# zwyang6/ExCEL

Hardware: AMD Instinct MI355X
Metric: images/sec (CAM+PAR refine, 448x448) (higher is better)
Workload: dtype bf16x3 (fp32 as bf16 hi+lo, fp32 accumulate)

## Files before the change

excel_amd/csrc/attn.hip:

```cpp
#include <stdlib.h>
#include "common.h"
#include "excel_internal.h"

namespace EXCEL_SPLIT_NS {

#define HD 64

struct RowpassArgs {
    float* out;
    float2* stats;
    int B, H, N;
    float scale;
    const unsigned short* qkvs;
    int flash_nq;
    int xcd_local;
    int tail_grp;
};

typedef unsigned short u16;

template <bool FLASH>
__device__ __forceinline__ void rowpass_body_bf(const RowpassArgs& p, float* smem, int b, int h, int type, int qblk) {
    constexpr int KT_EL = 32 * 128;
    constexpr int VSUB = 1152;
    constexpr int VT_EL = 8 * VSUB / 2;
    constexpr int STAGE_EL = KT_EL + (FLASH ? VT_EL : 0);
    constexpr int PER_WAVE = FLASH ? 4 : 2;
    const int tid = threadIdx.x, lane = tid & 63;
    const int wave = __builtin_amdgcn_readfirstlane(tid >> 6);
    const int r = lane & 31, kh = lane >> 5;
    const int N = p.N;
    const int tx = (type == 0 || type == 1) ? 0 : (type == 2 ? 1 : 2);
    const int ty = (type == 0) ? 1 : tx;
    const u16* Xsp = p.qkvs + (((long long)b * 3 + tx) * p.H + h) * (long long)N * 128;
    const u16* Ysp = p.qkvs + (((long long)b * 3 + ty) * p.H + h) * (long long)N * 128;
    const u16* Vsp = p.qkvs + (((long long)b * 3 + 2) * p.H + h) * (long long)N * 128;
    u16* ring = reinterpret_cast<u16*>(smem);
    const unsigned ring_b = __builtin_amdgcn_readfirstlane(lds_addr(ring));

    const int q0 = qblk * 128 + wave * 32;
    const int qrow = min(q0 + r, N - 1);
    splitx8 xh[4], xl[4];
#pragma unroll
    for (int s4 = 0; s4 < 4; ++s4) {
        xh[s4] = *reinterpret_cast<const splitx8*>(Xsp + (long long)qrow * 128 + s4 * 16 + kh * 8);
        xl[s4] = *reinterpret_cast<const splitx8*>(Xsp + (long long)qrow * 128 + 64 + s4 * 16 + kh * 8);
    }

    asm volatile("" : "+v"(xh[0]), "+v"(xh[1]), "+v"(xh[2]), "+v"(xh[3]), "+v"(xl[0]), "+v"(xl[1]), "+v"(xl[2]), "+v"(xl[3]));
    typedef __attribute__((address_space(3))) unsigned char* lds_bptr;
    const long long kplane_bytes = (long long)N * 256;
    const long long kavail = ((((long long)p.B * 3 - ((long long)b * 3 + ty)) * p.H - h) * kplane_bytes);
    const __amdgpu_buffer_rsrc_t rs_k = __builtin_amdgcn_make_buffer_rsrc((void*)Ysp, 0, (int)(kavail < (1LL << 31) - 1 ? kavail : (1LL << 31) - 1), 0x00020000);
    const long long vavail = ((((long long)p.B * 3 - ((long long)b * 3 + 2)) * p.H - h) * kplane_bytes);
    const __amdgpu_buffer_rsrc_t rs_v = __builtin_amdgcn_make_buffer_rsrc((void*)Vsp, 0, FLASH ? (int)(vavail < (1LL << 31) - 1 ? vavail : (1LL << 31) - 1) : 0, 0x00020000);
    int koffb[2], voffb[2];
#pragma unroll
    for (int j = 0; j < 2; ++j) {
        const int krow = wave * 8 + j * 4 + (lane >> 4);
        koffb[j] = krow * 256 + (((lane & 15) ^ (krow & 15)) * 16);
        const int sub = wave * 2 + j;
        voffb[j] = (lane >> 1) * 256 + (sub >> 2) * 128 + (((sub & 3) * 16 + (lane & 1) * 8) * 2);
    }
    auto issue_piece = [&](int kt, int stage, int idx) {
        unsigned dstk = __builtin_amdgcn_readfirstlane(ring_b + stage * (STAGE_EL * 2));
        asm volatile("" : "+s"(dstk));
        if (idx < 2) {
            __builtin_amdgcn_raw_ptr_buffer_load_lds(rs_k, (lds_bptr)(unsigned long long)(dstk + (wave * 8 + idx * 4) * 256), 16, koffb[idx], kt * (32 * 256), 0, 0);
        } else if (FLASH) {
            const int j = idx - 2;
            __builtin_amdgcn_raw_ptr_buffer_load_lds(rs_v, (lds_bptr)(unsigned long long)(dstk + KT_EL * 2 + (wave * 2 + j) * VSUB), 16, voffb[j], kt * (32 * 256), 0, 0);
        }
    };
    auto issue = [&](int kt, int stage) {
#pragma unroll
        for (int idx = 0; idx < PER_WAVE; ++idx) issue_piece(kt, stage, idx);
    };

    const float c2 = p.scale * 1.4426950408889634f;
    float m = -INFINITY, l = 0.f;
    f32x16 oT[2];
#pragma unroll
    for (int e = 0; e < 16; ++e) { oT[0][e] = 0.f; oT[1][e] = 0.f; }

    const int nkt = (N + 31) / 32;
    issue(0, 0);
    if (nkt > 1) issue(1, 1);
    int stage = 0;
    for (int kt = 0; kt < nkt; ++kt) {
        if (kt + 1 < nkt) {
            if (PER_WAVE == 4) asm volatile("s_waitcnt vmcnt(4)" ::: "memory");
            else asm volatile("s_waitcnt vmcnt(2)" ::: "memory");
        } else {
            asm volatile("s_waitcnt vmcnt(0)" ::: "memory");
        }
        __builtin_amdgcn_s_barrier();
        const int rstage = stage == 0 ? 2 : stage - 1;
        const bool refill = kt + 2 < nkt;
        if (q0 >= N) {
            if (refill) issue(kt + 2, rstage);
            stage = (stage == 2) ? 0 : stage + 1;
            continue;
        }
        const unsigned kr = ring_b + (stage * STAGE_EL + r * 128) * 2;
        f32x16 s;
#pragma unroll
        for (int e = 0; e < 16; ++e) s[e] = 0.f;
        {
            splitx8 yh[4], yl[4];
#pragma unroll
            for (int s4 = 0; s4 < 4; ++s4) {
                yh[s4] = lds_read16(kr + (((s4 * 2 + kh) ^ (r & 15)) * 16));
                yl[s4] = lds_read16(kr + (((8 + s4 * 2 + kh) ^ (r & 15)) * 16));
            }
            lds_wait8(yh, yl);
#pragma unroll
            for (int s4 = 0; s4 < 4; ++s4) {
                if (refill && s4 < PER_WAVE) issue_piece(kt + 2, rstage, s4);
                s = EXCEL_MFMA16(yl[s4], xh[s4], s, 0, 0, 0);
                s = EXCEL_MFMA16(yh[s4], xl[s4], s, 0, 0, 0);
                s = EXCEL_MFMA16(yh[s4], xh[s4], s, 0, 0, 0);
                __builtin_amdgcn_sched_barrier(0);
            }
        }
        if (kt == nkt - 1) {
#pragma unroll
            for (int e = 0; e < 16; ++e)
                if (kt * 32 + c32_row(e, lane) >= N) s[e] = -INFINITY;
        }
        float mx = s[0];
#pragma unroll
        for (int e = 1; e < 16; ++e) mx = fmaxf(mx, s[e]);
        {
            float mlo, mhi;
            wave_halves(mx, mlo, mhi);
            mx = fmaxf(mlo, mhi) * c2;
        }
        const float m_new = fmaxf(m, mx);
        const bool grew = m_new > m;
        const float alpha = __builtin_amdgcn_exp2f(m - m_new);
        float ps = 0.f;
#pragma unroll
        for (int e = 0; e < 16; ++e) {
            s[e] = __builtin_amdgcn_exp2f(fmaf(s[e], c2, -m_new));
            ps += s[e];
        }
        {
            float plo, phi;
            wave_halves(ps, plo, phi);
            ps = plo + phi;
        }
        l = l * alpha + ps;
        m = m_new;
        if (FLASH) {
            if (__any(grew)) {
#pragma unroll
                for (int e = 0; e < 16; ++e) { oT[0][e] *= alpha; oT[1][e] *= alpha; }
            }
            splitx8 ph[2], pl[2];
#ifdef EXCEL_SPLIT_F16
            {
                unsigned phu[2][4], plu[2][4];
#pragma unroll
                for (int e = 0; e < 16; e += 2) split_pair_bounded(s[e], s[e + 1], phu[e >> 3][(e & 7) >> 1], plu[e >> 3][(e & 7) >> 1]);
#pragma unroll
                for (int q = 0; q < 2; ++q) {
                    ph[q] = __builtin_bit_cast(splitx8, uint4{phu[q][0], phu[q][1], phu[q][2], phu[q][3]});
                    pl[q] = __builtin_bit_cast(splitx8, uint4{plu[q][0], plu[q][1], plu[q][2], plu[q][3]});
                }
            }
#else
#pragma unroll
            for (int e = 0; e < 16; ++e) {
                const float hf = __uint_as_float(__float_as_uint(s[e]) & 0xFFFF0000u);
                ph[e >> 3][e & 7] = split_hi(hf);
                pl[e >> 3][e & 7] = split_hi(s[e] - hf);
            }
#endif
            const unsigned vb = ring_b + (stage * STAGE_EL + KT_EL) * 2 + ((lane >> 4) & 1) * VSUB + (4 * kh + ((lane & 15) >> 2)) * 32 + (lane & 3) * 8;
#pragma unroll
            for (int dt = 0; dt < 2; ++dt) {
                splitx4 vq[8];
                const unsigned vbd = vb + dt * 2 * VSUB;
                vq[0] = lds_read8h_tr<0>(vbd);
                vq[1] = lds_read8h_tr<256>(vbd);
                vq[2] = lds_read8h_tr<4 * VSUB>(vbd);
                vq[3] = lds_read8h_tr<4 * VSUB + 256>(vbd);
                vq[4] = lds_read8h_tr<512>(vbd);
                vq[5] = lds_read8h_tr<512 + 256>(vbd);
                vq[6] = lds_read8h_tr<4 * VSUB + 512>(vbd);
                vq[7] = lds_read8h_tr<4 * VSUB + 512 + 256>(vbd);
                asm volatile("s_waitcnt lgkmcnt(0)" : "+v"(vq[0]), "+v"(vq[1]), "+v"(vq[2]), "+v"(vq[3]), "+v"(vq[4]), "+v"(vq[5]), "+v"(vq[6]), "+v"(vq[7])::"memory");
#pragma unroll
                for (int ks = 0; ks < 2; ++ks) {
                    const splitx4 h0 = vq[ks * 4], h1 = vq[ks * 4 + 1], l0 = vq[ks * 4 + 2], l1 = vq[ks * 4 + 3];
                    const splitx8 vh = {h0[0], h0[1], h0[2], h0[3], h1[0], h1[1], h1[2], h1[3]};
                    const splitx8 vl = {l0[0], l0[1], l0[2], l0[3], l1[0], l1[1], l1[2], l1[3]};
                    oT[dt] = EXCEL_MFMA16(vl, ph[ks], oT[dt], 0, 0, 0);
                    oT[dt] = EXCEL_MFMA16(vh, pl[ks], oT[dt], 0, 0, 0);
                    oT[dt] = EXCEL_MFMA16(vh, ph[ks], oT[dt], 0, 0, 0);
                }
            }
        }
        stage = (stage == 2) ? 0 : stage + 1;
    }

    const float linv = 1.f / l;
    if (kh == 0 && q0 + r < N)
        p.stats[(((long long)b * p.H + h) * 4 + type) * N + q0 + r] = make_float2(m, linv);

    if (FLASH) {
        __syncthreads();
        float* ob = smem + wave * (32 * 65);
#pragma unroll
        for (int dt = 0; dt < 2; ++dt)
#pragma unroll
            for (int e = 0; e < 16; ++e) ob[r * 65 + dt * 32 + c32_row(e, lane)] = oT[dt][e] * linv;
        __builtin_amdgcn_s_waitcnt(0xc07f);
        for (int qq = 0; qq < 32; ++qq) {
            const int q = q0 + qq;
            if (q >= N) break;
            const float v = ob[qq * 65 + lane];
            const split_t hi = split_hi(v);
            split_t* o = reinterpret_cast<split_t*>(p.out) + ((long long)b * N + q) * 2 * (p.H * HD) + split_off(h * HD + lane, 0);
            o[0] = hi;
            o[32] = split_hi(v - (float)hi);
        }
    }
}

__global__ __launch_bounds__(256, 2) void attn_rowpass_kernel(RowpassArgs p) {
    __shared__ __attribute__((aligned(1024))) float smem[3 * (2048 + 2304)];
    int bh, qb;
    rowpass_block_map(p.N, p.xcd_local, p.tail_grp, bh, qb);
    const int b = bh / p.H, h = bh % p.H;
    const int type = blockIdx.z;
    if (type == 0 && qb < p.flash_nq) rowpass_body_bf<true>(p, smem, b, h, 0, qb);
    else rowpass_body_bf<false>(p, smem, b, h, type, qb);
}

struct AccumArgs {
    const float2* stats;
    float* a_sum;
    float* w_aff;
    float* attn_out;
    int B, H, N, NP;
    float scale;
    float w_scale;
    float aff_scale;
    int aff_init;
    const unsigned short* qkvs;
    int dbg;
    const float* ex_attn;
    float ex_scale;
};

template <bool SURGERY>
__global__ __launch_bounds__(512, 2) void attn_accum_bf_kernel(AccumArgs p) {
    constexpr int XT = 128 * 128, YT = 64 * 128;
    constexpr int NTYPE = SURGERY ? 4 : 1;
    constexpr int TILES_EL = SURGERY ? 3 * XT + 3 * YT : 2 * (XT + YT);
    __shared__ __attribute__((aligned(1024))) u16 tiles[TILES_EL];
    __shared__ __attribute__((aligned(1024))) float2 lstats[2 * NTYPE * 128 + 32];
    const int tid = threadIdx.x, lane = tid & 63;
    const int wave = __builtin_amdgcn_readfirstlane(tid >> 6);
    const int r = lane & 31, kh = lane >> 5;
    const int wq = wave >> 1, wk = wave & 1;
    int kt = blockIdx.x, qt = blockIdx.y, b = blockIdx.z;
    if (EXCEL_DBG(p.dbg) & 8) {
        const int lin = blockIdx.x + gridDim.x * (blockIdx.y + gridDim.y * blockIdx.z);
        const int id = xcd_remap(lin, gridDim.x * gridDim.y * gridDim.z);
        kt = id % gridDim.x; qt = (id / gridDim.x) % gridDim.y; b = id / (gridDim.x * gridDim.y);
    }
    const int N = p.N;

    int rowx[4], coffx[4], rowy[2], coffy[2];
#pragma unroll
    for (int j = 0; j < 4; ++j) {
        const int row_l = wave * 16 + j * 4 + (lane >> 4);
        coffx[j] = ((lane & 15) ^ (row_l & 15)) * 8;
        rowx[j] = min(qt * 128 + row_l, N - 1);
    }
#pragma unroll
    for (int j = 0; j < 2; ++j) {
        const int row_l = wave * 8 + j * 4 + (lane >> 4);
        coffy[j] = ((lane & 15) ^ (row_l & 15)) * 8;
        rowy[j] = min(kt * 64 + row_l, N - 1);
    }
    auto issue_x = [&](int off, int typ, int h) {
        const u16* src = p.qkvs + (((long long)b * 3 + typ) * p.H + h) * (long long)N * 128;
#pragma unroll
        for (int j = 0; j < 4; ++j)
            __builtin_amdgcn_global_load_lds((const __attribute__((address_space(1))) void*)(src + (long long)rowx[j] * 128 + coffx[j]),
                                             (__attribute__((address_space(3))) void*)(tiles + off + (wave * 16 + j * 4) * 128), 16, 0, 0);
    };
    auto issue_y = [&](int off, int typ, int h) {
        const u16* src = p.qkvs + (((long long)b * 3 + typ) * p.H + h) * (long long)N * 128;
#pragma unroll
        for (int j = 0; j < 2; ++j)
            __builtin_amdgcn_global_load_lds((const __attribute__((address_space(1))) void*)(src + (long long)rowy[j] * 128 + coffy[j]),
                                             (__attribute__((address_space(3))) void*)(tiles + off + (wave * 8 + j * 4) * 128), 16, 0, 0);
    };
    auto issue_stats = [&](int h) {
        float* dst = reinterpret_cast<float*>(lstats + (h & 1) * NTYPE * 128);
#pragma unroll
        for (int j = 0; j < 2; ++j) {
            const int piece = wave * 2 + j;
            if (SURGERY || piece < 4) {
                const int ty = piece >> 2, q32 = (piece & 3) * 32 + (lane >> 1);
                const float* src = reinterpret_cast<const float*>(p.stats + (((long long)b * p.H + h) * 4 + ty) * N + min(qt * 128 + q32, N - 1)) + (lane & 1);
                __builtin_amdgcn_global_load_lds((const __attribute__((address_space(1))) void*)src,
                                                 (__attribute__((address_space(3))) void*)(dst + piece * 64), 4, 0, 0);
            } else {
                const float* src = reinterpret_cast<const float*>(p.stats + (((long long)b * p.H + h) * 4) * N + min(qt * 128 + (lane >> 1), N - 1)) + (lane & 1);
                __builtin_amdgcn_global_load_lds((const __attribute__((address_space(1))) void*)src,
                                                 (__attribute__((address_space(3))) void*)(reinterpret_cast<float*>(lstats) + 2 * NTYPE * 256), 4, 0, 0);
            }
        }
    };

    f32x16 accW, accA;
#pragma unroll
    for (int e = 0; e < 16; ++e) { accW[e] = 0.f; accA[e] = 0.f; }
    const float c2 = p.scale * 1.4426950408889634f;
    const bool last_kt = kt * 64 + wk * 32 + 32 > N;

    const bool tile_oob = (qt * 128 + wq * 32 >= N) || (kt * 64 + wk * 32 >= N);
    auto score = [&](int offY, int offX, int type, int h, f32x16& acc) {
        if ((EXCEL_DBG(p.dbg) & 1) || tile_oob) return;
        const float2 ml = lstats[((h & 1) * NTYPE + type) * 128 + wq * 32 + r];
        const u16* y16 = tiles + offY + (wk * 32 + r) * 128;
        const u16* x16 = tiles + offX + (wq * 32 + r) * 128;
        f32x16 s;
#pragma unroll
        for (int e = 0; e < 16; ++e) s[e] = 0.f;
#pragma unroll
        for (int s4 = 0; s4 < 4; ++s4) {
            const int ch = ((s4 * 2 + kh) ^ (r & 15)) * 8, cl = ((8 + s4 * 2 + kh) ^ (r & 15)) * 8;
            const splitx8 yh = *reinterpret_cast<const splitx8*>(y16 + ch), yl = *reinterpret_cast<const splitx8*>(y16 + cl);
            const splitx8 xh = *reinterpret_cast<const splitx8*>(x16 + ch), xl = *reinterpret_cast<const splitx8*>(x16 + cl);
            s = EXCEL_MFMA16(yl, xh, s, 0, 0, 0);
            s = EXCEL_MFMA16(yh, xl, s, 0, 0, 0);
            s = EXCEL_MFMA16(yh, xh, s, 0, 0, 0);
        }
        if (last_kt) {
#pragma unroll
            for (int e = 0; e < 16; ++e) {
                const int key = kt * 64 + wk * 32 + c32_row(e, lane);
                const float pr = __builtin_amdgcn_exp2f(fmaf(s[e], c2, -ml.x));
                acc[e] += (key < N) ? pr * ml.y : 0.f;
            }
        } else {
#pragma unroll
            for (int e = 0; e < 16; ++e) acc[e] = fmaf(__builtin_amdgcn_exp2f(fmaf(s[e], c2, -ml.x)), ml.y, acc[e]);
        }
    };

    if (SURGERY) {
        constexpr int XQ = 0, XK = XT, XV = 2 * XT, YQ = 3 * XT, YK = 3 * XT + YT, YV = 3 * XT + 2 * YT;
        issue_y(YQ, 0, 0);
        issue_stats(0);
        issue_x(XQ, 0, 0);
        issue_x(XK, 1, 0);
        issue_y(YK, 1, 0);
        for (int h = 0; h < p.H; ++h) {
            const bool more = h + 1 < p.H && !(EXCEL_DBG(p.dbg) & 2);
            asm volatile("s_waitcnt vmcnt(6)" ::: "memory");
            __builtin_amdgcn_s_barrier();
            if (!(EXCEL_DBG(p.dbg) & 2) || h == 0) { issue_x(XV, 2, h); issue_y(YV, 2, h); }
            score(YQ, XQ, 1, h, accA);
            if (!(EXCEL_DBG(p.dbg) & 2) || h == 0) asm volatile("s_waitcnt vmcnt(6)" ::: "memory");
            __builtin_amdgcn_s_barrier();
            if (more) { issue_y(YQ, 0, h + 1); issue_stats(h + 1); }
            score(YK, XQ, 0, h, accW);
            __builtin_amdgcn_s_barrier();
            if (more) issue_x(XQ, 0, h + 1);
            score(YK, XK, 2, h, accA);
            if (more) asm volatile("s_waitcnt vmcnt(8)" ::: "memory");
            else asm volatile("s_waitcnt vmcnt(0)" ::: "memory");
            __builtin_amdgcn_s_barrier();
            if (more) { issue_x(XK, 1, h + 1); issue_y(YK, 1, h + 1); }
            score(YV, XV, 3, h, accA);
        }
    } else {
        issue_x(0, 0, 0);
        issue_y(XT, 1, 0);
        issue_stats(0);
        for (int h = 0; h < p.H; ++h) {
            asm volatile("s_waitcnt vmcnt(0)" ::: "memory");
            __builtin_amdgcn_s_barrier();
            const int cur = (h & 1) * (XT + YT), nxt = (XT + YT) - cur;
            if (h + 1 < p.H) { issue_x(nxt, 0, h + 1); issue_y(nxt + XT, 1, h + 1); issue_stats(h + 1); }
            score(cur + XT, cur, 0, h, accW);
        }
    }
    __syncthreads();
    if (EXCEL_DBG(p.dbg) & 4) { if (accA[0] + accW[0] == 12345.f) p.a_sum[0] = 1.f; return; }

    float* tb = reinterpret_cast<float*>(tiles) + wave * (32 * 33);
    const int qbase = qt * 128 + wq * 32, kbase = kt * 64 + wk * 32;
    auto emit = [&](const f32x16& acc, int which) {
#pragma unroll
        for (int e = 0; e < 16; ++e) tb[r * 33 + c32_row(e, lane)] = acc[e];
        __builtin_amdgcn_s_waitcnt(0xc07f);
        float oldw[16];
        if (which == 1 && p.w_aff && !p.aff_init) {
#pragma unroll
            for (int i = 0; i < 16; ++i) {
                const int qg = qbase + 2 * i + kh, kg = kbase + r;
                const long long P = N - 1;
                oldw[i] = (qg < N && qg >= 1 && kg >= 1 && kg < N) ? p.w_aff[((long long)b * P + (qg - 1)) * P + (kg - 1)] : 0.f;
            }
        } else {
#pragma unroll
            for (int i = 0; i < 16; ++i) oldw[i] = 0.f;
        }
#pragma unroll
        for (int i = 0; i < 16; ++i) {
            const int qq = 2 * i + kh;
            const int qg = qbase + qq, kg = kbase + r;
            const float v = tb[qq * 33 + r];
            if (qg >= N) continue;
            if (which == 0) {
                if (kg < p.NP) {
                    float av = v * (1.f / 3.f);
                    if (p.ex_attn && qg >= 1 && kg >= 1 && kg < N) av += p.ex_scale * p.ex_attn[((long long)b * (N - 1) + (qg - 1)) * (N - 1) + (kg - 1)];
                    split_t* o = reinterpret_cast<split_t*>(p.a_sum) + ((long long)b * N + qg) * 2 * p.NP + split_off(kg, 0);
                    const split_t hi = split_hi(av);
                    o[0] = hi;
                    o[32] = split_hi(av - (float)hi);
                }
            } else {
                const float pw = v * p.w_scale;
                if (p.attn_out && kg < N) p.attn_out[((long long)b * N + qg) * N + kg] = pw;
                if (p.w_aff && qg >= 1 && kg >= 1 && kg < N) {
                    const long long P = N - 1;
                    p.w_aff[((long long)b * P + (qg - 1)) * P + (kg - 1)] = oldw[i] + pw * p.aff_scale;
                }
            }
        }
        __builtin_amdgcn_s_waitcnt(0xc07f);
    };
    if (SURGERY) emit(accA, 0);
    emit(accW, 1);
}

int excel_launch_attn_rowpass(const unsigned short* qkvs, float* out, float* stats, int B, int H, int N, int hd, float scale,
                              const AttnPlan& pl, hipStream_t st, int flash_nq) {
    ProfScope prof__(PROF_ATTN_ROWPASS, st);
    EXCEL_CHECK_ARG(hd == HD, "attention: head_dim must be 64 (got %d)", hd);
    EXCEL_CHECK_ARG(pl.rp_ntypes == 1 || pl.rp_ntypes == 4, "attention: ntypes must be 1 or 4");
    EXCEL_CHECK_ARG(pl.path != ATTN_TWOPASS_F32 && qkvs, "attention: the plan is of another mode");
    RowpassArgs a{out, reinterpret_cast<float2*>(stats), B, H, N, scale, qkvs, flash_nq, 1, 1 << 20};
#ifdef EXCEL_DEV
    { static const int x = getenv("EXCEL_ROWPASS_XCD") ? atoi(getenv("EXCEL_ROWPASS_XCD")) : 1; a.xcd_local = x; }
    { static const int g = getenv("EXCEL_ROWPASS_GRP") ? atoi(getenv("EXCEL_ROWPASS_GRP")) : 0; if (g > 0) a.tail_grp = g; }
#endif
    hipLaunchKernelGGL(attn_rowpass_kernel, dim3(pl.rp_grid[0], pl.rp_grid[1], pl.rp_grid[2]), dim3(256), 0, st, a);
    EXCEL_CHECK_LAUNCH("attn_rowpass");
    return EXCEL_OK;
}

int excel_launch_attn_accum(const unsigned short* qkvs, const float* stats, float* a_sum, float* w_aff, float* attn_out, int B, int H,
                            int N, int NP, int hd, float scale, int surgery, float w_scale, float aff_scale, int aff_init,
                            const AttnPlan& pl, hipStream_t st, const float* ex_attn) {
    ProfScope prof__(PROF_ATTN_ACCUM, st);
    EXCEL_CHECK_ARG(hd == HD, "attention: head_dim must be 64 (got %d)", hd);
    EXCEL_CHECK_ARG(pl.path == ATTN_TWOPASS_SPLIT && pl.block > 0 && qkvs, "attn_accum: the plan names another path");
    EXCEL_CHECK_ARG(!surgery || (a_sum && NP >= N && NP <= cdiv(N, 64) * 64), "attn_accum: bad a_sum/NP");
    AccumArgs a{reinterpret_cast<const float2*>(stats), a_sum, w_aff, attn_out, B, H, N, NP, scale, w_scale, aff_scale, aff_init, qkvs, 0, surgery ? ex_attn : nullptr, (float)H};
    const dim3 grid(pl.grid[0], pl.grid[1], pl.grid[2]), block(pl.block);
#ifdef EXCEL_DEV
    { static const char* d = getenv("EXCEL_ACCUM_DBG"); if (d) a.dbg = atoi(d); }
#endif
    if (surgery) hipLaunchKernelGGL((attn_accum_bf_kernel<true>), grid, block, 0, st, a);
    else hipLaunchKernelGGL((attn_accum_bf_kernel<false>), grid, block, 0, st, a);
    EXCEL_CHECK_LAUNCH("attn_accum");
    return EXCEL_OK;
}

}
```

Before: 1482.

## Prefetch V tiles before softmax, use max3 reductions, vectorize flash output stores

In the flash path, the transposed LDS reads of the V tile for both dt halves are issued before the row-max/exp softmax math, with one wait placed just before the PV MFMAs. This hides LDS latency behind the softmax ALU work. The row max now uses raw v_max3_f32/v_max_f32 inline asm, which skips fmaxf's NaN canonicalization. The epilogue now writes 16-byte vector stores of packed hi/lo pairs per lane instead of scalar per-element stores. In exchange, holding the V registers longer raises VGPR pressure and may cost occupancy.

```diff
diff --git a/excel_amd/csrc/attn.hip b/excel_amd/csrc/attn.hip
--- a/excel_amd/csrc/attn.hip
+++ b/excel_amd/csrc/attn.hip
@@ -18,6 +18,22 @@
 };
 
 typedef unsigned short u16;
+
+__device__ __forceinline__ float max_raw(float a, float b) {
+    float d;
+    asm("v_max_f32 %0, %1, %2" : "=v"(d) : "v"(a), "v"(b));
+    return d;
+}
+__device__ __forceinline__ float max3_raw(float a, float b, float c) {
+    float d;
+    asm("v_max3_f32 %0, %1, %2, %3" : "=v"(d) : "v"(a), "v"(b), "v"(c));
+    return d;
+}
+__device__ __forceinline__ void lds_wait16h(splitx4 (&a)[2][8]) {
+    asm volatile("s_waitcnt lgkmcnt(0)"
+                 : "+v"(a[0][0]), "+v"(a[0][1]), "+v"(a[0][2]), "+v"(a[0][3]), "+v"(a[0][4]), "+v"(a[0][5]), "+v"(a[0][6]), "+v"(a[0][7]),
+                   "+v"(a[1][0]), "+v"(a[1][1]), "+v"(a[1][2]), "+v"(a[1][3]), "+v"(a[1][4]), "+v"(a[1][5]), "+v"(a[1][6]), "+v"(a[1][7])::"memory");
+}
 
 template <bool FLASH>
 __device__ __forceinline__ void rowpass_body_bf(const RowpassArgs& p, float* smem, int b, int h, int type, int qblk) {
@@ -128,15 +144,32 @@
             for (int e = 0; e < 16; ++e)
                 if (kt * 32 + c32_row(e, lane) >= N) s[e] = -INFINITY;
         }
-        float mx = s[0];
-#pragma unroll
-        for (int e = 1; e < 16; ++e) mx = fmaxf(mx, s[e]);
+        splitx4 vq[2][8];
+        if (FLASH) {
+            const unsigned vb = ring_b + (stage * STAGE_EL + KT_EL) * 2 + ((lane >> 4) & 1) * VSUB + (4 * kh + ((lane & 15) >> 2)) * 32 + (lane & 3) * 8;
+#pragma unroll
+            for (int dt = 0; dt < 2; ++dt) {
+                const unsigned vbd = vb + dt * 2 * VSUB;
+                vq[dt][0] = lds_read8h_tr<0>(vbd);
+                vq[dt][1] = lds_read8h_tr<256>(vbd);
+                vq[dt][2] = lds_read8h_tr<4 * VSUB>(vbd);
+                vq[dt][3] = lds_read8h_tr<4 * VSUB + 256>(vbd);
+                vq[dt][4] = lds_read8h_tr<512>(vbd);
+                vq[dt][5] = lds_read8h_tr<512 + 256>(vbd);
+                vq[dt][6] = lds_read8h_tr<4 * VSUB + 512>(vbd);
+                vq[dt][7] = lds_read8h_tr<4 * VSUB + 512 + 256>(vbd);
+            }
+        }
+        float mx = max3_raw(s[0], s[1], s[2]);
+#pragma unroll
+        for (int e = 3; e < 15; e += 2) mx = max3_raw(mx, s[e], s[e + 1]);
+        mx = max_raw(mx, s[15]);
         {
             float mlo, mhi;
             wave_halves(mx, mlo, mhi);
-            mx = fmaxf(mlo, mhi) * c2;
-        }
-        const float m_new = fmaxf(m, mx);
+            mx = max_raw(mlo, mhi) * c2;
+        }
+        const float m_new = max_raw(m, mx);
         const bool grew = m_new > m;
         const float alpha = __builtin_amdgcn_exp2f(m - m_new);
         float ps = 0.f;
@@ -177,23 +210,12 @@
                 pl[e >> 3][e & 7] = split_hi(s[e] - hf);
             }
 #endif
-            const unsigned vb = ring_b + (stage * STAGE_EL + KT_EL) * 2 + ((lane >> 4) & 1) * VSUB + (4 * kh + ((lane & 15) >> 2)) * 32 + (lane & 3) * 8;
+            lds_wait16h(vq);
 #pragma unroll
             for (int dt = 0; dt < 2; ++dt) {
-                splitx4 vq[8];
-                const unsigned vbd = vb + dt * 2 * VSUB;
-                vq[0] = lds_read8h_tr<0>(vbd);
-                vq[1] = lds_read8h_tr<256>(vbd);
-                vq[2] = lds_read8h_tr<4 * VSUB>(vbd);
-                vq[3] = lds_read8h_tr<4 * VSUB + 256>(vbd);
-                vq[4] = lds_read8h_tr<512>(vbd);
-                vq[5] = lds_read8h_tr<512 + 256>(vbd);
-                vq[6] = lds_read8h_tr<4 * VSUB + 512>(vbd);
-                vq[7] = lds_read8h_tr<4 * VSUB + 512 + 256>(vbd);
-                asm volatile("s_waitcnt lgkmcnt(0)" : "+v"(vq[0]), "+v"(vq[1]), "+v"(vq[2]), "+v"(vq[3]), "+v"(vq[4]), "+v"(vq[5]), "+v"(vq[6]), "+v"(vq[7])::"memory");
 #pragma unroll
                 for (int ks = 0; ks < 2; ++ks) {
-                    const splitx4 h0 = vq[ks * 4], h1 = vq[ks * 4 + 1], l0 = vq[ks * 4 + 2], l1 = vq[ks * 4 + 3];
+                    const splitx4 h0 = vq[dt][ks * 4], h1 = vq[dt][ks * 4 + 1], l0 = vq[dt][ks * 4 + 2], l1 = vq[dt][ks * 4 + 3];
                     const splitx8 vh = {h0[0], h0[1], h0[2], h0[3], h1[0], h1[1], h1[2], h1[3]};
                     const splitx8 vl = {l0[0], l0[1], l0[2], l0[3], l1[0], l1[1], l1[2], l1[3]};
                     oT[dt] = EXCEL_MFMA16(vl, ph[ks], oT[dt], 0, 0, 0);
@@ -217,14 +239,20 @@
 #pragma unroll
             for (int e = 0; e < 16; ++e) ob[r * 65 + dt * 32 + c32_row(e, lane)] = oT[dt][e] * linv;
         __builtin_amdgcn_s_waitcnt(0xc07f);
-        for (int qq = 0; qq < 32; ++qq) {
+        const int d8 = lane & 7;
+        split_t* const obase = reinterpret_cast<split_t*>(p.out) + split_off(h * HD + d8 * 8, 0);
+#pragma unroll
+        for (int it = 0; it < 4; ++it) {
+            const int qq = it * 8 + (lane >> 3);
             const int q = q0 + qq;
-            if (q >= N) break;
-            const float v = ob[qq * 65 + lane];
-            const split_t hi = split_hi(v);
-            split_t* o = reinterpret_cast<split_t*>(p.out) + ((long long)b * N + q) * 2 * (p.H * HD) + split_off(h * HD + lane, 0);
-            o[0] = hi;
-            o[32] = split_hi(v - (float)hi);
+            unsigned hi2[4], lo2[4];
+#pragma unroll
+            for (int j = 0; j < 4; ++j) split_pair(ob[qq * 65 + d8 * 8 + 2 * j], ob[qq * 65 + d8 * 8 + 2 * j + 1], hi2[j], lo2[j]);
+            if (q < N) {
+                split_t* o = obase + ((long long)b * N + q) * 2 * (p.H * HD);
+                *reinterpret_cast<uint4*>(o) = uint4{hi2[0], hi2[1], hi2[2], hi2[3]};
+                *reinterpret_cast<uint4*>(o + 32) = uint4{lo2[0], lo2[1], lo2[2], lo2[3]};
+            }
         }
     }
 }
```

Result: no change. 1487, median of 6 (+0.4%).
